# Ignaciagothe/tda-eeg-audio

Measured on AMD Instinct MI355X. Metric: windows/sec end-to-end (dist->Rips H0/H1->Wasserstein), 47-ch EEG, higher is better.
Workload: dtype f64; 1 GPU; configs[4]+configs[2]: 1416 recordings x 5 bands x 15 selected windows = 106200 (EEG 47x250 f64, audio 250 f64) window pairs per pass, the whole job; per pair corr->dist->Rips H0/H1 (EEG 47 pts), tau per recording-band, Takens dim 3 sub 2 + Rips (audio, 23..123 pts over the bands), Wasserstein H0+H1, features, per-recording reductions; one all-gather of the (1416, 5x48) rows per pass; windows_per_pass=106200, windows_per_gpu_per_pass=106200, input_bytes_per_gpu=10195200000, batches_per_pass=1, windows_per_batch=106200, parallelism=recordings dealt over 1 rank(s), one all-gather per pass, batches_in_flight=3, hip_graph=True, batches_rerun_with_full_ladder=0

## Files before the change

### tda_eeg_audio_amd/csrc/rips.hip

```cpp
#include "common.h"
#include "corr_dist_dev.h"
#include <stdlib.h>

#ifndef CLOUD_NB
#define CLOUD_NB 8192
#endif
#ifndef NARROW_NT
#define NARROW_NT 512
#endif
#ifndef NARROW_WAVES
#define NARROW_WAVES 6
#endif
#if defined(TDA_PROFILE) && !defined(TDA_PROFILE_STOPS_ONLY)
#define NARROW_NB (NARROW_NT == 384 ? 1536 : 1024)
#else
#define NARROW_NB (NARROW_NT == 384 ? 1536 : 2048)
#endif
#define NARROW_EMAX 7626
#define NT_MAX 512
#define RANK_NONE 0x7fffu

#ifdef TDA_PROFILE
__device__ unsigned long long g_prof[48];
#ifdef TDA_PROFILE_STOPS_ONLY
// ... 82 lines not shown
{
    WT o = 0;
#pragma unroll
    for (int i = 0; i < W; ++i) o |= a.w[i];
    return o != 0;
}
template <int W, typename WT>
__device__ __forceinline__ Psi<W, WT> pzero()
{
    Psi<W, WT> r;
#pragma unroll
    for (int i = 0; i < W; ++i) r.w[i] = 0;
    return r;
}

__device__ __forceinline__ double wave_min_f64(double v)
{
#pragma unroll
    for (int off = 32; off > 0; off >>= 1) { const double o = __shfl_xor(v, off, 64); v = o < v ? o : v; }
    return v;
}
__device__ __forceinline__ double wave_max_f64(double v)
{
#pragma unroll
    for (int off = 32; off > 0; off >>= 1) { const double o = __shfl_xor(v, off, 64); v = o > v ? o : v; }
    return v;
}

__device__ __forceinline__ int tri2(int v) { return (v * (v - 1)) >> 1; }
__device__ __forceinline__ int pair_index(int x, int y) { return x > y ? tri2(x) + y : tri2(y) + x; }

__device__ __forceinline__ int edge_row(int e)
{
    const int a = (int)((1.0f + __builtin_amdgcn_sqrtf(1.0f + 8.0f * (float)e)) * 0.5f);
    const int t = tri2(a);
    return a + (t + a <= e ? 1 : 0) - (t > e ? 1 : 0);
}

#ifndef TDA_NO_EDGE_TABLE
struct EdgeTable {
    u16 v[8192 + 512];
    constexpr EdgeTable() : v()
    {
        int a = 1, b = 0;
        for (int e = 0; e < 8192 + 512; ++e) { v[e] = (u16)((a << 8) | b); if (++b == a) { ++a; b = 0; } }
    }
};
__device__ const EdgeTable g_edge_ab = EdgeTable();
__device__ __forceinline__ u32 edge_ab(int e) { return (u32)g_edge_ab.v[e]; }
#else
__device__ __forceinline__ u32 edge_ab(int e) { const int a = edge_row(e); return (u32)((a << 8) | (e - tri2(a))); }
#endif

struct WgVote {
    u32* slots;
    int parity;
};
template <int NT>
__device__ __forceinline__ bool wg_any(WgVote& v, bool p)
{
    static_assert(NT % 64 == 0 && NT <= 512, "slots are read as one or two 16-byte words; slots beyond NT / 64 hold zero");
    const bool w = __ballot(p) != 0ull;
    u32* s = v.slots + 8 * v.parity;
    if ((threadIdx.x & 63) == 0) s[threadIdx.x >> 6] = w ? 1u : 0u;
    __syncthreads();
    v.parity ^= 1;
    const uint4 x = *reinterpret_cast<const uint4*>(s);
    u32 r = x.x | x.y | x.z | x.w;
    if (NT > 256) { const uint4 y = *reinterpret_cast<const uint4*>(s + 4); r |= y.x | y.y | y.z | y.w; }
    return r != 0u;
}
template <int NT>
__device__ __forceinline__ bool wg_all(WgVote& v, bool p) { return !wg_any<NT>(v, !p); }

__device__ __forceinline__ int wave_incl_scan_i32(int v)
{
#define TDA_DPP_ADD_(CTRL, RM) v += __builtin_amdgcn_update_dpp(0, v, CTRL, RM, 0xF, true)
    TDA_DPP_ADD_(0x111, 0xF);
    TDA_DPP_ADD_(0x112, 0xF);
    TDA_DPP_ADD_(0x114, 0xF);
    TDA_DPP_ADD_(0x118, 0xF);
    TDA_DPP_ADD_(0x142, 0xA);
    TDA_DPP_ADD_(0x143, 0xC);
#undef TDA_DPP_ADD_
    return v;
}

__device__ __forceinline__ int edge_flat(u32 pk) { return tri2((int)(pk >> 8)) + (int)(pk & 255u); }

struct Bucketer {
    float dmin, scale, top;
    __device__ __forceinline__ int operator()(u32 key) const
    {
        const float x = fminf((sortable_f32(key) - dmin) * scale, top);
        const int b = (int)x;
        return b < 0 ? 0 : b;
    }
};

template <int NT>
__device__ __forceinline__ void effective_threshold(int n, u32 tkey, const u32* vmax, u32 kmin_thread, u32* red, u32& teff_out, u32& kmin_out)
{
    const int tid = threadIdx.x;
    const int lane = tid & 63;
    const u32 m0 = lane < n ? vmax[lane] : 0xffffffffu, m1 = lane + 64 < n ? vmax[lane + 64] : 0xffffffffu;
    const u32 renc = wave_min_u32_dpp(m0 < m1 ? m0 : m1);
    teff_out = renc < tkey ? renc : tkey;
    if (tid == 0) red[1] = 0xffffffffu;
    __syncthreads();
    const u32 kmin = wave_min_u32_dpp(kmin_thread);
    if (lane == 63) atomicMin(&red[1], kmin);
    __syncthreads();
    kmin_out = red[1];
}

template <int NT, int NB, bool WANT_KEYS>
__device__ __forceinline__ int rank_edges(const u32* key32, int E, u32 teff, u32 kmin, u16* members, u32* cursor, int* wsum, u16* rank,
                          u16* ord, u32* skey)
{
    static_assert(NB % (2 * NT) == 0, "every thread scans whole words");
    constexpr int WPT = NB / NT / 2;
    const int tid = threadIdx.x, lane = tid & 63, wave = tid >> 6;
    Bucketer bk;
    bk.dmin = sortable_f32(kmin);
    bk.top = (float)(NB - 1);
    bk.scale = bk.top / (sortable_f32(teff) - bk.dmin);
    for (int i = tid; i < NB / 2; i += NT) cursor[i] = 0u;
    __syncthreads();
#pragma unroll 4
    for (int e = tid; e < E; e += NT) {
        const u32 k = key32[e];
        u32 b = 0xffffu;
        if (k <= teff) { b = (u32)bk(k); atomicAdd(&cursor[b >> 1], 1u << (16 * (b & 1))); }
        rank[e] = (u16)b;
    }
    __syncthreads();
    {
        u32 w[WPT];
        int s = 0;
#pragma unroll
        for (int i = 0; i < WPT; ++i) {
// ... 205 lines not shown
#endif
#define TDA_SOLO_BEGIN() __builtin_amdgcn_s_setprio(TDA_SOLO_PRIO)
#define TDA_SOLO_END() __builtin_amdgcn_s_setprio(0)

#define TDA_POLL_LIMIT (1 << 16)
#ifndef TDA_TURN_SLEEP
#define TDA_TURN_SLEEP 4
#endif
#ifdef TDA_DEBUG_PTS
__device__ int g_fault;
extern "C" __attribute__((visibility("default"))) int tda_debug_inject(int what)
{
    return hipMemcpyToSymbol(HIP_SYMBOL(g_fault), &what, sizeof(int)) != hipSuccess;
}
#define TDA_FAULT(n) (g_fault == (n))
#else
#define TDA_FAULT(n) false
#endif
#ifdef TDA_DEBUG_PTS
#define GUARD_BYTES 16
__device__ __forceinline__ void guard_write(unsigned char* smem, const RipsLayout& L)
{
    if ((int)threadIdx.x < 4 * L.n_guard) reinterpret_cast<u32*>(smem + L.guard[threadIdx.x >> 2] - GUARD_BYTES)[threadIdx.x & 3] = 0xC0FFEE00u + threadIdx.x;
    __syncthreads();
}
__device__ __forceinline__ int guard_check(unsigned char* smem, const RipsLayout& L)
{
    __syncthreads();
    bool bad = false;
    if ((int)threadIdx.x < 4 * L.n_guard) bad = reinterpret_cast<u32*>(smem + L.guard[threadIdx.x >> 2] - GUARD_BYTES)[threadIdx.x & 3] != 0xC0FFEE00u + threadIdx.x;
    return __syncthreads_or(bad ? 1 : 0) ? TDA_WIN_LDS_GUARD : 0;
}
#else
#define GUARD_BYTES 0
__device__ __forceinline__ void guard_write(unsigned char*, const RipsLayout&) {}
__device__ __forceinline__ int guard_check(unsigned char*, const RipsLayout&) { return 0; }
#endif

#define MISC_COMP 0
#define MISC_CAND 512
#define MISC_WV (512 + 128)
#define MISC_MIN (512 + 192)
#define MISC_DONE (512 + 208)
#define MISC_SORTCNT (512 + 224)
#define MISC_SHARED (MISC_DONE + NT_MAX)
#define MISC_CKEY (MISC_SHARED + 96)
#define MISC_LIST MISC_CKEY
#define MISC_LIST_BYTES (4 * NT_MAX + 1280)
#define MISC_ADJ (MISC_LIST + MISC_LIST_BYTES)
#define MISC_ADJC (MISC_ADJ + 128 * 16)
#define MISC_BRANK (MISC_ADJC + 128 * 16)
#define MISC_BYTES(ncls) (MISC_BRANK + 8 * (ncls))

template <int NT, int NVW, int W, typename WT, bool NARROW, class KEYFN>
__device__ __forceinline__ void rips_sweep(int n, int E, int Ev, const u16* rank, const u16* ord, Psi<W, WT>* psi, int psi_bytes,
                           unsigned char* misc, KEYFN keyfn, double* h0, int h0_cap, double* h1, int h1_cap,
                           int& out_k0, int& out_k1, int& out_status)
{
    static_assert(!NARROW || W == 1, "the narrow layout is the point-cloud first pass");
    int psi_cap = 0;
    const int tid0 = threadIdx.x;
    const int lane0 = tid0 & 63, wave = uni(tid0 >> 6);
    int* brank = reinterpret_cast<int*>(misc + MISC_BRANK);
    u64* cand = reinterpret_cast<u64*>(misc + MISC_CAND);
    unsigned char* done = misc + MISC_DONE;
    SweepShared* shared = reinterpret_cast<SweepShared*>(misc + MISC_SHARED);
    u64* adj = reinterpret_cast<u64*>(misc + MISC_ADJ);
    constexpr int WB = 8 * (int)sizeof(WT);
    float* bkey = reinterpret_cast<float*>(misc + MISC_BRANK + 4 * WB * W);
    u64* adjc = reinterpret_cast<u64*>(misc + MISC_ADJC);

    if constexpr (!NARROW) for (int e = tid0; e < E; e += NT) psi[e] = pzero<W, WT>();
    for (int i = tid0; i < WB * W; i += NT) { brank[i] = -1; bkey[i] = 0.f; }
    for (int i = tid0; i < 256; i += NT) { adj[i] = 0ull; adjc[i] = 0ull; }
    if (tid0 == 0) {
        u32* lc = reinterpret_cast<u32*>(misc + MISC_MIN);
        lc[0] = 0u; lc[1] = 0xffffffffu; lc[2] = 0u;
        lc[3] = 0u;
        shared->status = 0;
    }
    if (tid0 < 16) {
        reinterpret_cast<u32*>(misc + MISC_WV)[tid0] = 0u;
        cand[tid0] = 0ull;
    }
    __syncthreads();

    WgVote vote{reinterpret_cast<u32*>(misc + MISC_WV), 0};
    WT alive[W];
#pragma unroll
    for (int c = 0; c < W; ++c) alive[c] = 0;
    int k0 = 0, k1 = 0, merges = 0, status = 0;
    int compA = lane0, compB = lane0 + 64;

    int clen = NT;
    int ordcls = 0;
    int cov_next = tid0;
#ifdef TDA_PROFILE
    int prof_rneed = 0, prof_chunk = -1;
#endif
    PROF_RESUME();
    for (int r0 = 0; r0 < Ev && !status; r0 += clen) {
        int tid = tid0;
        LAUNDER(tid);
        const int lane = tid & 63;
        clen = NT;
        PROF_MARK(15);
#ifdef TDA_PROFILE
        ++prof_chunk;
#endif
        PROF_COUNT(23, 1);
        const int r = r0 + tid;
        const bool valid = r < Ev;
        int a = 1, b = 0;
        if (valid) { const u32 pk = ord[r]; a = (int)(pk >> 8); b = (int)(pk & 255u); }
        const int tab = tri2(a) + b;
        const int slot = NARROW ? r : tab;
        if constexpr (NARROW) {
            psi_cap = (psi_bytes - 2 * (E - r0)) >> 2;
            if (r < psi_cap) psi[r] = pzero<W, WT>();
        }
        u64 M[NVW], M0[NVW];
        u64 Aj[NVW], Bj[NVW];
#pragma unroll
        for (int w = 0; w < NVW; ++w) { M[w] = 0; M0[w] = 0; Aj[w] = 0; Bj[w] = 0; }
        if (valid) {
#pragma unroll
            for (int w = 0; w < NVW; ++w) { Aj[w] = adj[2 * a + w]; Bj[w] = adj[2 * b + w]; M0[w] = Aj[w] & Bj[w]; }
        }
        {
            volatile u32* turn = reinterpret_cast<volatile u32*>(misc + MISC_MIN) + 2;
            if (wave > 0) {
                int trips = 0;
                for (;;) {
                    const u32 t = (u32)uni((int)*turn);
                    if (t >= (u32)wave) break;
                    if (++trips > TDA_POLL_LIMIT) { if (lane == 0) turn[1] = 1u; break; }
                    if (t + 1u < (u32)wave) __builtin_amdgcn_s_sleep(TDA_TURN_SLEEP); else __builtin_amdgcn_s_sleep(0);
                }
            }
            __builtin_amdgcn_fence(__ATOMIC_ACQUIRE, "workgroup");
            if (valid) {
#pragma unroll
                for (int w = 0; w < NVW; ++w) M[w] = (Aj[w] | adjc[2 * a + w]) & (Bj[w] | adjc[2 * b + w]);
                atomicOr(reinterpret_cast<unsigned long long*>(&adjc[2 * a + (b >> 6)]), 1ull << (b & 63));
                atomicOr(reinterpret_cast<unsigned long long*>(&adjc[2 * b + (a >> 6)]), 1ull << (a & 63));
            }
            LDS_ORDER();
            if (lane == 0 && !(TDA_FAULT(1) && wave == 3)) *turn = (u32)wave + 1u;
        }
        if (valid) {
            const int ta0 = tri2(a), tb0 = tri2(b);
#pragma unroll
            for (int w = 0; w < NVW; ++w) {
                u64 cc = (Aj[w] | adjc[2 * a + w]) & (Bj[w] | adjc[2 * b + w]) & ~M[w];
                while (cc) {
                    const int v0 = 64 * w + __builtin_ctzll(cc); cc &= cc - 1ull;
                    const bool ok1 = cc != 0ull; const int v1 = ok1 ? 64 * w + __builtin_ctzll(cc) : v0; cc &= cc - 1ull;
                    const int t0 = tri2(v0), t1 = tri2(v1);
                    const u32 xa0 = rank[v0 < a ? ta0 + v0 : t0 + a], xb0 = rank[v0 < b ? tb0 + v0 : t0 + b];
                    const u32 xa1 = rank[v1 < a ? ta0 + v1 : t1 + a], xb1 = rank[v1 < b ? tb0 + v1 : t1 + b];
                    if ((int)(xa0 > xb0 ? xa0 : xb0) < r) M[w] |= 1ull << (v0 & 63);
                    if (ok1 && (int)(xa1 > xb1 ? xa1 : xb1) < r) M[w] |= 1ull << (v1 & 63);
                }
            }
        }
        u64 many = 0;
#pragma unroll
        for (int w = 0; w < NVW; ++w) many |= M[w];
        const bool is_cand = valid && many == 0;
        int vstar = 0, d1 = 0, d2 = 0, q1 = 0, q2 = 0;
        {
            u64 many0 = 0;
#pragma unroll
            for (int w = 0; w < NVW; ++w) many0 |= M0[w];
            if (many0) {
                if (NVW == 1 || M0[0]) vstar = __builtin_ctzll(M0[0]);
                else vstar = 64 + __builtin_ctzll(M0[NVW - 1]);
            } else if (many) {
                if (NVW == 1 || M[0]) vstar = __builtin_ctzll(M[0]);
                else vstar = 64 + __builtin_ctzll(M[NVW - 1]);
            }
            if (valid && many != 0) {
                d1 = pair_index(a, vstar); d2 = pair_index(b, vstar);
                q1 = (int)rank[d1] - r0; q2 = (int)rank[d2] - r0;
                if (TDA_FAULT(2) && tid == 77 && q1 >= 0) q1 = tid;
            }
        }
        PROF_MARK(4);
        PROF_STOPC(11, out_k0 = k0; out_k1 = k1; out_status = 0);
        u64* mbal = reinterpret_cast<u64*>(misc + MISC_COMP);
        u64* zbal = mbal + 8;
        int* offs = reinterpret_cast<int*>(mbal + 16);
        u16* freebits = reinterpret_cast<u16*>(misc + MISC_CKEY);
        float mykey = 0.f;
        if (is_cand) mykey = keyfn(r, a, b);
        {
            const u64 bal = __ballot(is_cand), zb = __ballot(is_cand && mykey == 0.0f);
            if (lane == 0) { cand[wave] = bal; zbal[wave] = zb; }
        }
        done[tid] = 0;
        __syncthreads();
        PROF_MARK(21);
        PROF_STOPC(12, out_k0 = k0; out_k1 = k1; out_status = 0);
        int nfree = 0;
#pragma unroll
        for (int c = 0; c < W; ++c) nfree += __builtin_popcountll((u64)(WT)~alive[c]);
        int ncand = 0;
#pragma unroll
        for (int w = 0; w < NT / 64; ++w) ncand += __builtin_popcountll(cand[w]);
        int btot = 0;
        if (ncand > 0) {
        const bool par = ncand > 24;
        const int lblA0 = compA, lblB0 = compB;
        int qpar = NT;
        if (par) {
            int* bcomp = reinterpret_cast<int*>(misc + MISC_LIST + 1024);
            u32* bbest2 = reinterpret_cast<u32*>(bcomp + 128);
            int* bpar = reinterpret_cast<int*>(bcomp + 384);
            auto rounds = [&](int limit) {
                if (wave == 0) { bcomp[lane] = lblA0; bcomp[64 + lane] = lblB0; }
                if (tid < 256) bbest2[tid] = 0xffffffffu;
                __syncthreads();
                bool live = is_cand && tid < limit, picked = false;
                for (int round = 0; round < 64; ++round) {
                    u32* bbest = bbest2 + 128 * (round & 1);
                    int ca = 0, cb2 = 0;
                    if (live) {
                        ca = bcomp[a]; cb2 = bcomp[b];
                        if (ca == cb2) live = false;
                        else { atomicMin(&bbest[ca], (u32)tid); atomicMin(&bbest[cb2], (u32)tid); }
                    }
                    if (!wg_any<NT>(vote, live)) break;
                    if (live && (bbest[ca] == (u32)tid || bbest[cb2] == (u32)tid)) { picked = true; live = false; }
                    if (wave == 0) {
                        TDA_SOLO_BEGIN();
                        int pp[2];
#pragma unroll
                        for (int h = 0; h < 2; ++h) {
                            const int me = lane + 64 * h;
                            pp[h] = me;
                            const u32 bp = bbest[me];
                            if (bp != 0xffffffffu) {
                                const u32 pk = ord[r0 + (int)bp];
                                const int oa = bcomp[pk >> 8], ob = bcomp[pk & 255u];
                                pp[h] = oa == me ? ob : oa;
                                if (bbest[pp[h]] == bp && me < pp[h]) pp[h] = me;
                            }
                        }
                        bpar[lane] = pp[0]; bpar[64 + lane] = pp[1];
                        for (int it = 0; it < 8; ++it) {
                            const int p0 = bpar[lane], p1 = bpar[64 + lane];
                            const int g0 = bpar[p0], g1 = bpar[p1];
                            if (__ballot(g0 != p0 || g1 != p1) == 0ull) break;
                            bpar[lane] = g0; bpar[64 + lane] = g1;
                        }
                        const int c0 = bcomp[lane], c1 = bcomp[64 + lane];
                        const int n0 = bpar[c0], n1 = bpar[c1];
                        bcomp[lane] = n0; bcomp[64 + lane] = n1;
                        u32* other = bbest2 + 128 * ((round + 1) & 1);
                        other[lane] = 0xffffffffu; other[64 + lane] = 0xffffffffu;
                        TDA_SOLO_END();
                    }
                    __syncthreads();
                }
                const u64 mb = __ballot(picked);
                if (lane == 0) mbal[wave] = mb;
                __syncthreads();
            };
            rounds(NT);
            int nbirth = 0, wcut = -1, before = 0;
#pragma unroll
            for (int w = 0; w < NT / 64; ++w) {
                const int nb = __builtin_popcountll(cand[w] & ~mbal[w]);
                if (wcut < 0 && nbirth + nb > nfree) { wcut = w; before = nbirth; }
                nbirth += nb;
            }
            if (wcut >= 0) {
                u64 bw = cand[wcut] & ~mbal[wcut];
                for (int k = before; k < nfree; ++k) bw &= bw - 1ull;
                qpar = 64 * wcut + __builtin_ctzll(bw);
                PROF_COUNT(26, 1);
                __syncthreads();
                rounds(qpar);
            }
            if (wave == 0) { compA = bcomp[lane]; compB = bcomp[64 + lane]; }
        }
        if (wave == 0) {
            TDA_SOLO_BEGIN();
            const u64 candv = cand[lane & 7];
            int q = par ? qpar : NT, births = 0;
            const bool walk = !par;
            for (int g = 0; g < NT / 64 && walk; ++g) {
                u64 cb = q == NT ? rl64(candv, g) : 0ull;
                u64 mm = 0ull;
                if (cb) {
                    PROF_COUNT(20, __builtin_popcountll(cb));
                    const u32 pkv = ord[r0 + 64 * g + lane < E ? r0 + 64 * g + lane : E - 1];
                    while (cb) {
                        const int l = __builtin_ctzll(cb);
                        cb &= cb - 1;
                        const u32 pk = rl32(pkv, l);
                        const int qa = (int)(pk >> 8), qb = (int)(pk & 255u);
                        int ca, cbb;
                        if (NVW == 1) {
                            ca = (int)rl32((u32)compA, qa);
                            cbb = (int)rl32((u32)compA, qb);
                        } else {
                            const int a0 = (int)rl32((u32)compA, qa & 63), a1 = (int)rl32((u32)compB, qa & 63);
                            const int b0 = (int)rl32((u32)compA, qb & 63), b1 = (int)rl32((u32)compB, qb & 63);
                            ca = qa < 64 ? a0 : a1;
                            cbb = qb < 64 ? b0 : b1;
                        }
                        const bool same = ca == cbb, open = q == NT;
                        q = (open && same && births == nfree) ? 64 * g + l : q;
                        births += same ? 1 : 0;
                        const int cnew = (q == NT) ? ca : cbb;
                        compA = compA == cbb ? cnew : compA;
                        if (NVW == 2) compB = compB == cbb ? cnew : compB;
                        mm |= (!same && q == NT) ? (1ull << l) : 0ull;
                    }
                }
                if (lane == 0) mbal[g] = mm;
            }
            int nb = 0, nr = 0, nm = 0;
            if (lane < NT / 64) {
                u64 cg = cand[lane];
                if (64 * lane >= q) cg = 0ull;
                else if (q < 64 * lane + 64) cg &= (1ull << (q - 64 * lane)) - 1ull;
                const u64 mg = mbal[lane], zg = zbal[lane];
                nb = __builtin_popcountll(cg & ~mg); nr = __builtin_popcountll(mg & ~zg); nm = __builtin_popcountll(mg);
            }
            int pb = 0, pr = 0, tb = 0, tr = 0, tm = 0;
#pragma unroll
            for (int w = 0; w < NT / 64; ++w) {
                const int xb = (int)rl32((u32)nb, w), xr = (int)rl32((u32)nr, w), xm = (int)rl32((u32)nm, w);
                if (w < lane) { pb += xb; pr += xr; }
                tb += xb; tr += xr; tm += xm;
            }
            if (lane < NT / 64) { offs[lane] = pb; offs[8 + lane] = pr; }
            if (lane == 0) { offs[16] = tb; offs[17] = tr; offs[18] = tm; offs[19] = q; }
            TDA_SOLO_END();
        } else {
            for (int t = tid - 64; t < WB * W; t += NT - 64) {
                const int cw = t / WB, bit = t & (WB - 1);
                int rk = 0;
                bool fr = false;
#pragma unroll
                for (int c = 0; c < W; ++c) {
                    const WT f_ = (WT)~alive[c];
                    if (c < cw) rk += __builtin_popcountll((u64)f_);
                    if (c == cw) { rk += __builtin_popcountll((u64)(f_ & (((WT)1 << bit) - (WT)1))); fr = (f_ >> bit) & (WT)1; }
                }
                if (fr) freebits[rk] = (u16)t;
            }
        }
        __syncthreads();
        PROF_MARK(22);
        PROF_STOPC(13, out_k0 = k0; out_k1 = k1; out_status = 0);
        clen = uni(offs[19]);
        if (clen == 0) status |= TDA_WIN_CLASS_OVERFLOW;
        if (clen < NT) PROF_COUNT(14, 1);
        bool mrg = is_cand && ((mbal[wave] >> lane) & 1ull);
        bool birth = is_cand && !mrg && tid < clen;
        bool row = mrg && mykey != 0.0f;
        const u64 below = (1ull << lane) - 1ull;
        const int bpre = offs[wave] + __builtin_popcountll(__ballot(birth) & below);
        const int rpre = offs[8 + wave] + __builtin_popcountll(__ballot(row) & below);
        btot = uni(offs[16]);
        const int rtot = uni(offs[17]), mtot = uni(offs[18]);
        if (!status) {
            if (row) {
                const int pos = k0 + rpre;
                if (pos < h0_cap) { h0[2 * pos] = 0.0; h0[2 * pos + 1] = (double)mykey; }
            }
            k0 += rtot; merges += mtot;
            if (birth) {
                const int idx = (int)freebits[bpre];
                const int cw = idx / WB, bit = idx & (WB - 1);
                Psi<W, WT> nv = pzero<W, WT>();
#pragma unroll
                for (int c = 0; c < W; ++c)
                    if (c == cw) nv.w[c] = ((WT)1 << bit);
                if (!NARROW || r < psi_cap) psi[slot] = nv;
                brank[idx] = r;
                bkey[idx] = mykey;
            }
            if (W == 1 && wave == 0 && btot > 0) {
                const int nal = __builtin_popcountll((u64)alive[0]);
                if (lane >= nal && lane < nal + btot) ordcls = (int)freebits[lane - nal];
            }
            int left = btot;
#pragma unroll
            for (int c = 0; c < W; ++c) {
                const u64 f_ = (u64)(WT)~alive[c];
                const int pc = __builtin_popcountll(f_);
                if (left >= pc) { alive[c] = (WT)~(WT)0; left -= pc; }
                else if (left > 0) {
                    int lo = 0, hi = 63;
                    while (lo < hi) {
                        const int mid = (lo + hi) >> 1;
                        if (__builtin_popcountll(f_ & ((2ull << mid) - 1ull)) >= left) hi = mid; else lo = mid + 1;
                    }
                    alive[c] |= (WT)(f_ & ((2ull << lo) - 1ull));
                    left = 0;
                }
            }
        }
        }
        if (status) break;
        PROF_MARK(5);
        PROF_STOPC(14, out_k0 = k0; out_k1 = k1; out_status = 0);
        bool quiet = btot == 0;
#pragma unroll
        for (int c = 0; c < W; ++c) quiet = quiet && alive[c] == 0;
        u32* lcnt = reinterpret_cast<u32*>(misc + MISC_MIN);
        if (quiet) PROF_COUNT(24, 1);
#ifdef TDA_PROFILE
        if (!quiet) prof_rneed = r0 + clen;
#endif
        if constexpr (NARROW) {
            if (!quiet && r0 + NT > psi_cap) { status |= TDA_WIN_CLASS_OVERFLOW; break; }
        }
// ... 318 lines not shown
                    if (nk == KMAX) { more = 1; break; }
                    const int src = __builtin_ctzll(__ballot(mk == best));
                    Psi<W, WT> mine = pzero<W, WT>();
#pragma unroll
                    for (int q = 0; q < LPL; ++q)
                        if (q < nq && ek[q] == best) mine = ev[q];
                    Psi<W, WT> wv;
#pragma unroll
                    for (int c = 0; c < W; ++c) {
                        if (sizeof(WT) == 8) wv.w[c] = (WT)rl64((u64)mine.w[c], src);
                        else wv.w[c] = (WT)rl32((u32)mine.w[c], src);
                    }
                    const int rk = r0 + (int)(best >> 8);
                    int ybit, ycw;
                    float ybirth;
                    if (W == 1) {
                        const u64 ob = __ballot(lane < nalive0 && (((u64)wv.w[0] >> ordcls) & 1ull));
                        if (!ob) { status |= TDA_WIN_CLASS_OVERFLOW; break; }
                        const int opos = 63 - __builtin_clzll(ob);
                        ybit = (int)rl32((u32)ordcls, opos);
                        ycw = 0;
                        ybirth = __uint_as_float(rl32(__float_as_uint(bky[0]), ybit));
                        const int up = __builtin_amdgcn_update_dpp(0, ordcls, 0x130, 0xF, 0xF, true);
                        if (lane >= opos) ordcls = up;
                        --nalive0;
                    } else {
                        int candv = -1, cwl = 0;
                        float byl = 0.f;
#pragma unroll
                        for (int c = 0; c < W; ++c)
                            if (lane < WB && ((wv.w[c] >> lb) & (WT)1) && brk[c] > candv) { candv = brk[c]; cwl = c; byl = bky[c]; }
                        const int bestr = wave_max_i32_dpp(candv);
                        const u64 ybal = __ballot(candv == bestr && candv >= 0);
                        if (!ybal) { status |= TDA_WIN_CLASS_OVERFLOW; break; }
                        ybit = __builtin_ctzll(ybal);
                        ycw = (int)rl32((u32)cwl, ybit);
                        ybirth = __uint_as_float(rl32(__float_as_uint(byl), ybit));
                    }
                    if (FTAB) {
                        WT sel = 0;
#pragma unroll
                        for (int c = 0; c < W; ++c)
                            if (c == ycw) sel = (vimg.w[c] >> ybit) & (WT)1;
                        if (lane < nk && sel) vimg = pxor(vimg, wv);
                        if (lane == nk) {
                            vimg = wv;
#pragma unroll
                            for (int c = 0; c < W; ++c)
                                if (c == ycw) vimg.w[c] &= (WT)~((WT)1 << ybit);
                            mycode = ((u32)ycw << 8) | (u32)ybit; myrk = (u32)rk; mybirth = ybirth;
                        }
                    } else {
                        const u32 pkk = ord[rk];
                        const float key = keyfn(rk, (int)(pkk >> 8), (int)(pkk & 255u));
                        if (key > ybirth) {
                            if (k1 < h1_cap && lane == 0) { h1[2 * k1] = (double)ybirth; h1[2 * k1 + 1] = (double)key; }
                            ++k1;
                        }
                        if (lane == 0) {
                            *reinterpret_cast<u32*>(list + ES * nk) = ((u32)ycw << 8) | (u32)ybit;
#pragma unroll
                            for (int c = 0; c < W; ++c) *reinterpret_cast<WT*>(list + ES * nk + 4 + c * (int)sizeof(WT)) = wv.w[c];
                        }
                    }
#pragma unroll
                    for (int q = 0; q < LPL; ++q) {
                        if (q >= nq) break;
                        WT sel = 0;
#pragma unroll
                        for (int c = 0; c < W; ++c)
                            if (c == ycw) sel = (ev[q].w[c] >> ybit) & (WT)1;
                        if (sel) ev[q] = pxor(ev[q], wv);
                    }
#pragma unroll
                    for (int c = 0; c < W; ++c)
                        if (c == ycw) alive[c] &= (WT)~((WT)1 << ybit);
                    ++nk;
                }
                PROF_MARK(31);
                PROF_COUNT(10, nk);
                if (FTAB) {
                    const bool mine_ok = lane < nk;
                    float key = 0.f;
                    if (mine_ok) {
                        const u32 pkk = ord[(int)myrk];
                        key = keyfn((int)myrk, (int)(pkk >> 8), (int)(pkk & 255u));
                    }
                    const bool emit = mine_ok && key > mybirth;
                    const u64 bal = __ballot(emit);
                    const int pos = k1 + __builtin_popcountll(bal & ((1ull << lane) - 1ull));
                    if (emit && pos < h1_cap) { h1[2 * pos] = (double)mybirth; h1[2 * pos + 1] = (double)key; }
                    k1 += __builtin_popcountll(bal);
                    if (mine_ok) {
                        Psi<W, WT>* ftab = reinterpret_cast<Psi<W, WT>*>(list);
                        ftab[WB * (int)(mycode >> 8) + (int)(mycode & 255u)] = vimg;
                    }
                }
                if (lane == 0) {
#pragma unroll
                    for (int c = 0; c < W; ++c) shared->alive[c] = (u64)alive[c];
                    shared->k1 = k1; shared->nk = nk; shared->more = more; shared->status = status;
                }
                TDA_SOLO_END();
            }
            __syncthreads();
            PROF_MARK(18);
            PROF_STOPC(18, out_k0 = k0; out_k1 = k1; out_status = 0);
            WT kmask[W];
#pragma unroll
            for (int c = 0; c < W; ++c) {
                const WT na = sizeof(WT) == 8 ? (WT)uni64(shared->alive[c]) : (WT)uni((int)(u32)shared->alive[c]);
                kmask[c] = alive_before[c] & (WT)~na; alive[c] = na;
            }
            k1 = uni(shared->k1);
            const int nk = uni(shared->nk);
            const bool more = uni(shared->more) != 0;
            status = uni(shared->status);
            if (status) break;
            if (FTAB) {
                const Psi<W, WT>* ftab = reinterpret_cast<const Psi<W, WT>*>(list);
                const int seen_end = r0 + clen < Ev ? r0 + clen : Ev;
#pragma unroll 4
                for (int rr = tid; rr < seen_end; rr += NT) {
                    const int e = NARROW ? rr : edge_flat(ord[rr]);
                    const Psi<W, WT> p = psi[e];
                    WT anyh = 0;
#pragma unroll
                    for (int c = 0; c < W; ++c) anyh |= p.w[c] & kmask[c];
                    if (!anyh) continue;
                    Psi<W, WT> q;
#pragma unroll
                    for (int c = 0; c < W; ++c) q.w[c] = p.w[c] & (WT)~kmask[c];
#pragma unroll
                    for (int c = 0; c < W; ++c) {
                        u64 hh = (u64)(p.w[c] & kmask[c]);
                        while (hh) {
                            const int bit = __builtin_ctzll(hh);
                            hh &= hh - 1ull;
                            q = pxor(q, ftab[WB * c + bit]);
// ... 6 lines not shown
                    u32 kc[4];
                    Psi<W, WT> kw[4];
#pragma unroll
                    for (int j = 0; j < 4; ++j) {
                        const int jj = j0 + j < nk ? j0 + j : j0;
                        kc[j] = j0 + j < nk ? *reinterpret_cast<const u32*>(list + ES * jj) : 0xffffffffu;
#pragma unroll
                        for (int c = 0; c < W; ++c) kw[j].w[c] = *reinterpret_cast<const WT*>(list + ES * jj + 4 + c * (int)sizeof(WT));
                    }
#pragma unroll 4
                    for (int rr = tid; rr < (r0 + clen < Ev ? r0 + clen : Ev); rr += NT) {
                        const int e = NARROW ? rr : edge_flat(ord[rr]);
                        Psi<W, WT> p = psi[e];
                        bool changed = false;
#pragma unroll
                        for (int j = 0; j < 4; ++j) {
                            if (kc[j] == 0xffffffffu) continue;
                            const int jcw = (int)(kc[j] >> 8), jbit = (int)(kc[j] & 255u);
                            WT sel = 0;
#pragma unroll
                            for (int c = 0; c < W; ++c)
                                if (c == jcw) sel = (p.w[c] >> jbit) & (WT)1;
                            if (sel) { p = pxor(p, kw[j]); changed = true; }
                        }
                        if (changed) psi[e] = p;
                    }
                }
            }
            PROF_MARK(19);
            PROF_STOPC(19, out_k0 = k0; out_k1 = k1; out_status = 0);
            if (complete && !more) break;
            if (++list_rounds > 4 * NT) { status |= TDA_WIN_CLASS_OVERFLOW; break; }
            __syncthreads();
        }
        }
        if (valid && tid < clen) {
            atomicOr(reinterpret_cast<unsigned long long*>(&adj[2 * a + (b >> 6)]), 1ull << (b & 63));
            atomicOr(reinterpret_cast<unsigned long long*>(&adj[2 * b + (a >> 6)]), 1ull << (a & 63));
        }
        if (tid < 256) adjc[tid] = 0ull;
        if (tid == 0) {
            lcnt[0] = 0u; lcnt[1] = 0xffffffffu; lcnt[2] = 0u; shared->clen = 0x7fffffff;
            if (lcnt[3]) shared->status = TDA_WIN_NOT_CONVERGED;
        }
        __syncthreads();
        if (uni(shared->status) & TDA_WIN_NOT_CONVERGED) { status |= TDA_WIN_NOT_CONVERGED; break; }
        if (quiet) {
            const int from = r0 + clen;
            bool covered = true;
            int rr = (NT & (NT - 1)) == 0 ? from + ((tid - from) & (NT - 1)) : from + (((tid - from) % NT) + NT) % NT;
            rr = rr > cov_next ? rr : cov_next;
            while (rr < Ev) {
                const u32 pk = ord[rr];
                const int ea = (int)(pk >> 8), eb = (int)(pk & 255u);
                u64 common = adj[2 * ea] & adj[2 * eb];
                if (NVW == 2) common |= adj[2 * ea + 1] & adj[2 * eb + 1];
                if (common == 0ull) { covered = false; break; }
                rr += NT;
            }
            cov_next = rr;
            {
                const u32 wmin = wave_min_u32_dpp(covered ? 0x7fffffffu : (u32)rr);
                if (lane == 0 && wmin != 0x7fffffffu) atomicMin(reinterpret_cast<unsigned int*>(&shared->clen), wmin);
            }
            __syncthreads();
            const int ru = uni(shared->clen);
            if (ru >= Ev) { PROF_COUNT(25, 1); PROF_MARK(7); break; }
            if (ru > from) {
                for (int r2 = from + tid; r2 < ru; r2 += NT) {
                    const u32 pk = ord[r2];
                    const int ea = (int)(pk >> 8), eb = (int)(pk & 255u);
                    atomicOr(reinterpret_cast<unsigned long long*>(&adj[2 * ea + (eb >> 6)]), 1ull << (eb & 63));
                    atomicOr(reinterpret_cast<unsigned long long*>(&adj[2 * eb + (ea >> 6)]), 1ull << (ea & 63));
                    if constexpr (NARROW) { if (r2 < ((psi_bytes - 2 * (E - ru)) >> 2)) psi[r2] = pzero<W, WT>(); }
                }
                PROF_COUNT(35, ru - from);
                clen = ru - r0;
                __syncthreads();
            }
        }
        PROF_MARK(7);
        PROF_STOPC(20, out_k0 = k0; out_k1 = k1; out_status = 0);
    }
#ifdef TDA_PROFILE
    PROF_COUNT(36, prof_rneed > 4096 ? 1 : 0); PROF_COUNT(37, prof_rneed > 4608 ? 1 : 0); PROF_COUNT(38, prof_rneed > 5120 ? 1 : 0);
    PROF_COUNT(39, prof_rneed); PROF_COUNT(40, Ev);
#endif
    const int ncomp = n - merges;
    for (int i = 0; i < ncomp; ++i) {
        if (k0 < h0_cap && tid0 == 0) { h0[2 * k0] = 0.0; h0[2 * k0 + 1] = (double)INFINITY; }
        ++k0;
    }
#pragma unroll
    for (int c = 0; c < W; ++c) {
        u64 al = (u64)alive[c];
        while (al) {
            const int bit = __builtin_ctzll(al);
            al &= al - 1;
            if (k1 < h1_cap && tid0 == 0) { h1[2 * k1] = (double)bkey[WB * c + bit]; h1[2 * k1 + 1] = (double)INFINITY; }
            ++k1;
        }
    }
    if (k1 > h1_cap) status |= TDA_WIN_H1_TRUNCATED;
    out_k0 = k0; out_k1 = k1; out_status = status;
}


#define TOT_NW 128
#define TOT_SLOTS 8
#define TOT_SLOT_WORDS ((size_t)8128 * TOT_NW)

template <int NT, class KEYFN>
__device__ __forceinline__ void rips_sweep_total(int n, int E, int Ev, const u16* rank, const u16* ord, float* bkey, unsigned char* misc,
                                 u64* __restrict__ psi_g, KEYFN keyfn, double* h0, int h0_cap, double* h1, int h1_cap,
                                 int& out_k0, int& out_k1, int& out_status)
{
    constexpr int NWV = NT / 64;
    const int tid = threadIdx.x, lane = tid & 63, wave = uni(tid >> 6);
    u64* adj = reinterpret_cast<u64*>(misc + MISC_ADJ);
    int* comp = reinterpret_cast<int*>(misc + MISC_COMP);
    u32* flags = reinterpret_cast<u32*>(misc + MISC_WV);
    u64* yv = reinterpret_cast<u64*>(misc + MISC_LIST);
    u64* cur = yv + TOT_NW;
    u32* nzbit = reinterpret_cast<u32*>(misc + MISC_ADJ + 4096);
    u32* alivebit = nzbit + 256;
    static_assert(MISC_LIST_BYTES >= 2 * TOT_NW * 8, "scratch of the total sweep");
    for (int i = tid; i < 256; i += NT) { adj[i] = 0ull; nzbit[i] = 0u; alivebit[i] = 0u; }
    for (int v = tid; v < 128; v += NT) comp[v] = v;
    __syncthreads();
    int k0 = 0, k1 = 0, merges = 0, nborn = 0, nalive = 0;
    auto stored = [&](int rr) { return (nzbit[rr >> 5] >> (rr & 31)) & 1u; };
    for (int r = 0; r < Ev; ++r) {
        const u32 pk = (u32)uni((int)ord[r]);
        const int a = (int)(pk >> 8), b = (int)(pk & 255u);
        const u64 M0 = uni64(adj[2 * a] & adj[2 * b]), M1 = uni64(adj[2 * a + 1] & adj[2 * b + 1]);
        if ((M0 | M1) == 0ull) {
            const int ca = uni(comp[a]), cb = uni(comp[b]);
            const float key = keyfn(r, a, b);
            __syncthreads();
// ... 975 lines not shown
```

Baseline: 4.153 million windows/s.

## Precompute H0 spanning forest via Boruvka before sweep, drop per-chunk merge detection

```diff
diff --git a/tda_eeg_audio_amd/csrc/rips.hip b/tda_eeg_audio_amd/csrc/rips.hip
--- a/tda_eeg_audio_amd/csrc/rips.hip
+++ b/tda_eeg_audio_amd/csrc/rips.hip
@@ -158,27 +158,6 @@
 __device__ __forceinline__ u32 edge_ab(int e) { const int a = edge_row(e); return (u32)((a << 8) | (e - tri2(a))); }
 #endif
 
-struct WgVote {
-    u32* slots;
-    int parity;
-};
-template <int NT>
-__device__ __forceinline__ bool wg_any(WgVote& v, bool p)
-{
-    static_assert(NT % 64 == 0 && NT <= 512, "slots are read as one or two 16-byte words; slots beyond NT / 64 hold zero");
-    const bool w = __ballot(p) != 0ull;
-    u32* s = v.slots + 8 * v.parity;
-    if ((threadIdx.x & 63) == 0) s[threadIdx.x >> 6] = w ? 1u : 0u;
-    __syncthreads();
-    v.parity ^= 1;
-    const uint4 x = *reinterpret_cast<const uint4*>(s);
-    u32 r = x.x | x.y | x.z | x.w;
-    if (NT > 256) { const uint4 y = *reinterpret_cast<const uint4*>(s + 4); r |= y.x | y.y | y.z | y.w; }
-    return r != 0u;
-}
-template <int NT>
-__device__ __forceinline__ bool wg_all(WgVote& v, bool p) { return !wg_any<NT>(v, !p); }
-
 __device__ __forceinline__ int wave_incl_scan_i32(int v)
 {
 #define TDA_DPP_ADD_(CTRL, RM) v += __builtin_amdgcn_update_dpp(0, v, CTRL, RM, 0xF, true)
@@ -192,7 +171,7 @@
     return v;
 }
 
-__device__ __forceinline__ int edge_flat(u32 pk) { return tri2((int)(pk >> 8)) + (int)(pk & 255u); }
+__device__ __forceinline__ int edge_flat(u32 pk) { return tri2((int)((pk >> 8) & 127u)) + (int)(pk & 255u); }
 
 struct Bucketer {
     float dmin, scale, top;
@@ -504,17 +483,141 @@
 #define MISC_BRANK (MISC_ADJC + 128 * 16)
 #define MISC_BYTES(ncls) (MISC_BRANK + 8 * (ncls))
 
+#define TDA_WIN_FOREST_GUARD 0x200
+#define ORD_FOREST 0x8000u
+
+typedef unsigned short u16x2 __attribute__((ext_vector_type(2)));
+typedef short i16x2 __attribute__((ext_vector_type(2)));
+__device__ __forceinline__ u16x2 as_u16x2(u32 x) { return __builtin_bit_cast(u16x2, x); }
+
+template <int NT, int NVW>
+__device__ __forceinline__ int spanning_forest(int n, const u16* rank, u16* ord, unsigned char* misc)
+{
+    constexpr int NV = 64 * NVW;
+    constexpr int TPV = (NT / NV) >= 8 ? 8 : (NT / NV) >= 4 ? 4 : (NT / NV) >= 2 ? 2 : 1;
+    constexpr int UPT = NV / TPV;
+    static_assert(NT >= NV && UPT % 4 == 0, "one thread per vertex at least, whole label words");
+    unsigned char* flab = misc + MISC_LIST + 1024;
+    u32* fbest = reinterpret_cast<u32*>(flab + 128);
+    int* fhook = reinterpret_cast<int*>(flab + 640);
+    const int tid = threadIdx.x, lane = tid & 63, wave = tid >> 6;
+    const int v = tid / TPV, j = tid & (TPV - 1);
+    if (tid < 128) { flab[tid] = (unsigned char)tid; fbest[tid] = 0xffffffffu; }
+    u32 row[UPT / 2];
+    {
+        const int tv = tri2(v), u0 = UPT * j;
+        int tu = tri2(u0);
+#pragma unroll
+        for (int i = 0; i < UPT; ++i) {
+            const int u = u0 + i;
+            const bool ok = v < n && u < n && u != v;
+            const u32 rk = rank[ok ? (u < v ? tv + u : tu + v) : 0];
+            const u32 x = ok ? rk : RANK_NONE;
+            if (i & 1) row[i >> 1] |= x << 16; else row[i >> 1] = x;
+            tu += u;
+        }
+    }
+    __syncthreads();
+    int ncomp = n;
+    for (int round = 0; ncomp > 1; ++round) {
+        if (v < n) {
+            const int cv = flab[v];
+            u16x2 acc = {0xffffu, 0xffffu};
+            if (round == 0) {
+#pragma unroll
+                for (int k = 0; k < UPT / 2; ++k) acc = __builtin_elementwise_min(acc, as_u16x2(row[k]));
+            } else {
+                const u32 cv4 = (u32)cv * 0x01010101u;
+#pragma unroll
+                for (int k = 0; k < UPT / 4; ++k) {
+                    const u32 x4 = reinterpret_cast<const u32*>(flab + UPT * j)[k] ^ cv4;
+#pragma unroll
+                    for (int h = 0; h < 2; ++h) {
+                        const u16x2 d = as_u16x2(__builtin_amdgcn_perm(0u, x4, h ? 0x0c030c02u : 0x0c010c00u));
+                        const u16x2 one = {1u, 1u};
+                        const i16x2 same = __builtin_bit_cast(i16x2, (u16x2)(d - one)) >> (short)15;
+                        acc = __builtin_elementwise_min(acc, as_u16x2(row[2 * k + h] | __builtin_bit_cast(u32, same)));
+                    }
+                }
+            }
+            u32 m = acc.x < acc.y ? acc.x : acc.y;
+#pragma unroll
+            for (int s = 1; s < TPV; s <<= 1) {
+                const u32 o = (u32)__shfl_xor((int)m, s);
+                m = o < m ? o : m;
+            }
+            if (j == 0 && m < RANK_NONE) atomicMin(&fbest[cv], m);
+        }
+        __syncthreads();
+        if (wave == 0) {
+            TDA_SOLO_BEGIN();
+            int c[NVW], p[NVW];
+            bool hook[NVW];
+#pragma unroll
+            for (int h = 0; h < NVW; ++h) {
+                const int me = lane + 64 * h;
+                c[h] = flab[me];
+                p[h] = me;
+                hook[h] = false;
+                const u32 bm = fbest[me];
+                if (c[h] == me && bm != 0xffffffffu) {
+                    const u32 pk = ord[bm];
+                    const int la = flab[(pk >> 8) & 127u], lb = flab[pk & 255u];
+                    const int o = la == me ? lb : la;
+                    const bool root = fbest[o] == bm && me < o;
+                    if (!root) {
+                        p[h] = o;
+                        ord[bm] = (u16)(pk | ORD_FOREST);
+                        hook[h] = true;
+                    }
+                }
+            }
+#pragma unroll
+            for (int h = 0; h < NVW; ++h) fbest[lane + 64 * h] = 0xffffffffu;
+            for (;;) {
+                int g[NVW];
+                bool moved = false;
+#pragma unroll
+                for (int h = 0; h < NVW; ++h) {
+                    g[h] = __shfl(p[0], p[h] & 63);
+                    if (NVW == 2) { const int g1 = __shfl(p[NVW - 1], p[h] & 63); g[h] = p[h] < 64 ? g[h] : g1; }
+                    moved = moved || g[h] != p[h];
+                }
+                if (__ballot(moved) == 0ull) break;
+#pragma unroll
+                for (int h = 0; h < NVW; ++h) p[h] = g[h];
+            }
+#pragma unroll
+            for (int h = 0; h < NVW; ++h) {
+                int nc = __shfl(p[0], c[h] & 63);
+                if (NVW == 2) { const int n1 = __shfl(p[NVW - 1], c[h] & 63); nc = c[h] < 64 ? nc : n1; }
+                flab[lane + 64 * h] = (unsigned char)nc;
+            }
+            int hooks = 0;
+#pragma unroll
+            for (int h = 0; h < NVW; ++h) hooks += __builtin_popcountll(__ballot(hook[h]));
+            if (lane == 0) *fhook = hooks;
+            TDA_SOLO_END();
+        }
+        __syncthreads();
+        const int hooks = uni(*fhook);
+        PROF_COUNT(42, 1);
+        if (hooks == 0) break;
+        ncomp -= hooks;
+    }
+    return ncomp;
+}
+
 template <int NT, int NVW, int W, typename WT, bool NARROW, class KEYFN>
-__device__ __forceinline__ void rips_sweep(int n, int E, int Ev, const u16* rank, const u16* ord, Psi<W, WT>* psi, int psi_bytes,
+__device__ __forceinline__ void rips_sweep(int n, int E, int Ev, const u16* rank, u16* ord, Psi<W, WT>* psi, int psi_bytes,
                            unsigned char* misc, KEYFN keyfn, double* h0, int h0_cap, double* h1, int h1_cap,
                            int& out_k0, int& out_k1, int& out_status)
 {
     static_assert(!NARROW || W == 1, "the narrow layout is the point-cloud first pass");
     int psi_cap = 0;
     const int tid0 = threadIdx.x;
-    const int lane0 = tid0 & 63, wave = uni(tid0 >> 6);
+    const int wave = uni(tid0 >> 6);
     int* brank = reinterpret_cast<int*>(misc + MISC_BRANK);
-    u64* cand = reinterpret_cast<u64*>(misc + MISC_CAND);
     unsigned char* done = misc + MISC_DONE;
     SweepShared* shared = reinterpret_cast<SweepShared*>(misc + MISC_SHARED);
     u64* adj = reinterpret_cast<u64*>(misc + MISC_ADJ);
@@ -531,18 +634,12 @@
         lc[3] = 0u;
         shared->status = 0;
     }
-    if (tid0 < 16) {
-        reinterpret_cast<u32*>(misc + MISC_WV)[tid0] = 0u;
-        cand[tid0] = 0ull;
-    }
-    __syncthreads();
-
-    WgVote vote{reinterpret_cast<u32*>(misc + MISC_WV), 0};
+    __syncthreads();
+
     WT alive[W];
 #pragma unroll
     for (int c = 0; c < W; ++c) alive[c] = 0;
     int k0 = 0, k1 = 0, merges = 0, status = 0;
-    int compA = lane0, compB = lane0 + 64;
 
     int clen = NT;
     int ordcls = 0;
@@ -551,6 +648,12 @@
     int prof_rneed = 0, prof_chunk = -1;
 #endif
     PROF_RESUME();
+    const int fcomps = spanning_forest<NT, NVW>(n, rank, ord, misc);
+    (void)fcomps;
+#ifdef TDA_DEBUG_PTS
+    bool fguard = false;
+#endif
+    PROF_MARK(41);
     for (int r0 = 0; r0 < Ev && !status; r0 += clen) {
         int tid = tid0;
         LAUNDER(tid);
@@ -564,7 +667,8 @@
         const int r = r0 + tid;
         const bool valid = r < Ev;
         int a = 1, b = 0;
-        if (valid) { const u32 pk = ord[r]; a = (int)(pk >> 8); b = (int)(pk & 255u); }
+        bool forest = false;
+        if (valid) { const u32 pk = ord[r]; a = (int)((pk >> 8) & 127u); b = (int)(pk & 255u); forest = (pk & ORD_FOREST) != 0u; }
         const int tab = tri2(a) + b;
         const int slot = NARROW ? r : tab;
         if constexpr (NARROW) {
@@ -640,15 +744,31 @@
         }
         PROF_MARK(4);
         PROF_STOPC(11, out_k0 = k0; out_k1 = k1; out_status = 0);
-        u64* mbal = reinterpret_cast<u64*>(misc + MISC_COMP);
-        u64* zbal = mbal + 8;
-        int* offs = reinterpret_cast<int*>(mbal + 16);
+        u64* bbal = reinterpret_cast<u64*>(misc + MISC_COMP);
+        u64* rbal = bbal + 8;
+        u64* mbal = bbal + 16;
         u16* freebits = reinterpret_cast<u16*>(misc + MISC_CKEY);
         float mykey = 0.f;
         if (is_cand) mykey = keyfn(r, a, b);
+        const bool fmrg = valid && forest, fbirth = is_cand && !forest;
+#ifdef TDA_DEBUG_PTS
+        fguard = fguard || (fmrg && !is_cand);
+#endif
         {
-            const u64 bal = __ballot(is_cand), zb = __ballot(is_cand && mykey == 0.0f);
-            if (lane == 0) { cand[wave] = bal; zbal[wave] = zb; }
+            const u64 bb = __ballot(fbirth), rb = __ballot(fmrg && mykey != 0.0f), mb = __ballot(fmrg);
+            if (lane == 0) { bbal[wave] = bb; rbal[wave] = rb; mbal[wave] = mb; }
+        }
+        for (int t = tid; t < WB * W; t += NT) {
+            const int cw = t / WB, bit = t & (WB - 1);
+            int rk = 0;
+            bool fr = false;
+#pragma unroll
+            for (int c = 0; c < W; ++c) {
+                const WT f_ = (WT)~alive[c];
+                if (c < cw) rk += __builtin_popcountll((u64)f_);
+                if (c == cw) { rk += __builtin_popcountll((u64)(f_ & (((WT)1 << bit) - (WT)1))); fr = (f_ >> bit) & (WT)1; }
+            }
+            if (fr) freebits[rk] = (u16)t;
         }
         done[tid] = 0;
         __syncthreads();
@@ -657,169 +777,38 @@
         int nfree = 0;
 #pragma unroll
         for (int c = 0; c < W; ++c) nfree += __builtin_popcountll((u64)(WT)~alive[c]);
-        int ncand = 0;
-#pragma unroll
-        for (int w = 0; w < NT / 64; ++w) ncand += __builtin_popcountll(cand[w]);
+        const int wl = lane < NT / 64 ? lane : 0;
+        const u64 bv = lane < NT / 64 ? bbal[wl] : 0ull, rv = lane < NT / 64 ? rbal[wl] : 0ull, mv = lane < NT / 64 ? mbal[wl] : 0ull;
+        const int nbl = __builtin_popcountll(bv);
+        const int ibl = wave_incl_scan_i32(nbl);
+        const int nball = (int)rl32((u32)ibl, NT / 64 - 1);
         int btot = 0;
-        if (ncand > 0) {
-        const bool par = ncand > 24;
-        const int lblA0 = compA, lblB0 = compB;
-        int qpar = NT;
-        if (par) {
-            int* bcomp = reinterpret_cast<int*>(misc + MISC_LIST + 1024);
-            u32* bbest2 = reinterpret_cast<u32*>(bcomp + 128);
-            int* bpar = reinterpret_cast<int*>(bcomp + 384);
-            auto rounds = [&](int limit) {
-                if (wave == 0) { bcomp[lane] = lblA0; bcomp[64 + lane] = lblB0; }
-                if (tid < 256) bbest2[tid] = 0xffffffffu;
-                __syncthreads();
-                bool live = is_cand && tid < limit, picked = false;
-                for (int round = 0; round < 64; ++round) {
-                    u32* bbest = bbest2 + 128 * (round & 1);
-                    int ca = 0, cb2 = 0;
-                    if (live) {
-                        ca = bcomp[a]; cb2 = bcomp[b];
-                        if (ca == cb2) live = false;
-                        else { atomicMin(&bbest[ca], (u32)tid); atomicMin(&bbest[cb2], (u32)tid); }
-                    }
-                    if (!wg_any<NT>(vote, live)) break;
-                    if (live && (bbest[ca] == (u32)tid || bbest[cb2] == (u32)tid)) { picked = true; live = false; }
-                    if (wave == 0) {
-                        TDA_SOLO_BEGIN();
-                        int pp[2];
-#pragma unroll
-                        for (int h = 0; h < 2; ++h) {
-                            const int me = lane + 64 * h;
-                            pp[h] = me;
-                            const u32 bp = bbest[me];
-                            if (bp != 0xffffffffu) {
-                                const u32 pk = ord[r0 + (int)bp];
-                                const int oa = bcomp[pk >> 8], ob = bcomp[pk & 255u];
-                                pp[h] = oa == me ? ob : oa;
-                                if (bbest[pp[h]] == bp && me < pp[h]) pp[h] = me;
-                            }
-                        }
-                        bpar[lane] = pp[0]; bpar[64 + lane] = pp[1];
-                        for (int it = 0; it < 8; ++it) {
-                            const int p0 = bpar[lane], p1 = bpar[64 + lane];
-                            const int g0 = bpar[p0], g1 = bpar[p1];
-                            if (__ballot(g0 != p0 || g1 != p1) == 0ull) break;
-                            bpar[lane] = g0; bpar[64 + lane] = g1;
-                        }
-                        const int c0 = bcomp[lane], c1 = bcomp[64 + lane];
-                        const int n0 = bpar[c0], n1 = bpar[c1];
-                        bcomp[lane] = n0; bcomp[64 + lane] = n1;
-                        u32* other = bbest2 + 128 * ((round + 1) & 1);
-                        other[lane] = 0xffffffffu; other[64 + lane] = 0xffffffffu;
-                        TDA_SOLO_END();
-                    }
-                    __syncthreads();
-                }
-                const u64 mb = __ballot(picked);
-                if (lane == 0) mbal[wave] = mb;
-                __syncthreads();
-            };
-            rounds(NT);
-            int nbirth = 0, wcut = -1, before = 0;
-#pragma unroll
-            for (int w = 0; w < NT / 64; ++w) {
-                const int nb = __builtin_popcountll(cand[w] & ~mbal[w]);
-                if (wcut < 0 && nbirth + nb > nfree) { wcut = w; before = nbirth; }
-                nbirth += nb;
-            }
-            if (wcut >= 0) {
-                u64 bw = cand[wcut] & ~mbal[wcut];
-                for (int k = before; k < nfree; ++k) bw &= bw - 1ull;
-                qpar = 64 * wcut + __builtin_ctzll(bw);
-                PROF_COUNT(26, 1);
-                __syncthreads();
-                rounds(qpar);
-            }
-            if (wave == 0) { compA = bcomp[lane]; compB = bcomp[64 + lane]; }
-        }
-        if (wave == 0) {
-            TDA_SOLO_BEGIN();
-            const u64 candv = cand[lane & 7];
-            int q = par ? qpar : NT, births = 0;
-            const bool walk = !par;
-            for (int g = 0; g < NT / 64 && walk; ++g) {
-                u64 cb = q == NT ? rl64(candv, g) : 0ull;
-                u64 mm = 0ull;
-                if (cb) {
-                    PROF_COUNT(20, __builtin_popcountll(cb));
-                    const u32 pkv = ord[r0 + 64 * g + lane < E ? r0 + 64 * g + lane : E - 1];
-                    while (cb) {
-                        const int l = __builtin_ctzll(cb);
-                        cb &= cb - 1;
-                        const u32 pk = rl32(pkv, l);
-                        const int qa = (int)(pk >> 8), qb = (int)(pk & 255u);
-                        int ca, cbb;
-                        if (NVW == 1) {
-                            ca = (int)rl32((u32)compA, qa);
-                            cbb = (int)rl32((u32)compA, qb);
-                        } else {
-                            const int a0 = (int)rl32((u32)compA, qa & 63), a1 = (int)rl32((u32)compB, qa & 63);
-                            const int b0 = (int)rl32((u32)compA, qb & 63), b1 = (int)rl32((u32)compB, qb & 63);
-                            ca = qa < 64 ? a0 : a1;
-                            cbb = qb < 64 ? b0 : b1;
-                        }
-                        const bool same = ca == cbb, open = q == NT;
-                        q = (open && same && births == nfree) ? 64 * g + l : q;
-                        births += same ? 1 : 0;
-                        const int cnew = (q == NT) ? ca : cbb;
-                        compA = compA == cbb ? cnew : compA;
-                        if (NVW == 2) compB = compB == cbb ? cnew : compB;
-                        mm |= (!same && q == NT) ? (1ull << l) : 0ull;
-                    }
-                }
-                if (lane == 0) mbal[g] = mm;
-            }
-            int nb = 0, nr = 0, nm = 0;
-            if (lane < NT / 64) {
-                u64 cg = cand[lane];
-                if (64 * lane >= q) cg = 0ull;
-                else if (q < 64 * lane + 64) cg &= (1ull << (q - 64 * lane)) - 1ull;
-                const u64 mg = mbal[lane], zg = zbal[lane];
-                nb = __builtin_popcountll(cg & ~mg); nr = __builtin_popcountll(mg & ~zg); nm = __builtin_popcountll(mg);
-            }
-            int pb = 0, pr = 0, tb = 0, tr = 0, tm = 0;
-#pragma unroll
-            for (int w = 0; w < NT / 64; ++w) {
-                const int xb = (int)rl32((u32)nb, w), xr = (int)rl32((u32)nr, w), xm = (int)rl32((u32)nm, w);
-                if (w < lane) { pb += xb; pr += xr; }
-                tb += xb; tr += xr; tm += xm;
-            }
-            if (lane < NT / 64) { offs[lane] = pb; offs[8 + lane] = pr; }
-            if (lane == 0) { offs[16] = tb; offs[17] = tr; offs[18] = tm; offs[19] = q; }
-            TDA_SOLO_END();
-        } else {
-            for (int t = tid - 64; t < WB * W; t += NT - 64) {
-                const int cw = t / WB, bit = t & (WB - 1);
-                int rk = 0;
-                bool fr = false;
-#pragma unroll
-                for (int c = 0; c < W; ++c) {
-                    const WT f_ = (WT)~alive[c];
-                    if (c < cw) rk += __builtin_popcountll((u64)f_);
-                    if (c == cw) { rk += __builtin_popcountll((u64)(f_ & (((WT)1 << bit) - (WT)1))); fr = (f_ >> bit) & (WT)1; }
-                }
-                if (fr) freebits[rk] = (u16)t;
-            }
-        }
-        __syncthreads();
+        if (nball > 0 || __ballot(mv != 0ull) != 0ull) {
+        int q = NT;
+        const u64 over = __ballot(lane < NT / 64 && ibl > nfree);
+        if (over) {
+            const int wcut = __builtin_ctzll(over);
+            u64 bw = rl64(bv, wcut);
+            for (int k = (int)rl32((u32)(ibl - nbl), wcut); k < nfree; ++k) bw &= bw - 1ull;
+            q = 64 * wcut + __builtin_ctzll(bw);
+            PROF_COUNT(26, 1);
+        }
+        const u64 keep = 64 * lane + 64 <= q ? ~0ull : 64 * lane >= q ? 0ull : (1ull << (q - 64 * lane)) - 1ull;
+        const int pk3 = nbl | (__builtin_popcountll(rv & keep) << 10) | (__builtin_popcountll(mv & keep) << 20);
+        const int i3 = wave_incl_scan_i32(pk3);
+        const int before3 = wave > 0 ? (int)rl32((u32)i3, wave - 1) : 0, tot3 = (int)rl32((u32)i3, NT / 64 - 1);
+        const int pb = before3 & 1023, pr = (before3 >> 10) & 1023, rtot = (tot3 >> 10) & 1023, mtot = tot3 >> 20;
+        btot = over ? nfree : nball;
+        clen = q;
         PROF_MARK(22);
         PROF_STOPC(13, out_k0 = k0; out_k1 = k1; out_status = 0);
-        clen = uni(offs[19]);
         if (clen == 0) status |= TDA_WIN_CLASS_OVERFLOW;
         if (clen < NT) PROF_COUNT(14, 1);
-        bool mrg = is_cand && ((mbal[wave] >> lane) & 1ull);
-        bool birth = is_cand && !mrg && tid < clen;
-        bool row = mrg && mykey != 0.0f;
+        const bool birth = fbirth && tid < clen;
+        const bool row = fmrg && mykey != 0.0f && tid < clen;
         const u64 below = (1ull << lane) - 1ull;
-        const int bpre = offs[wave] + __builtin_popcountll(__ballot(birth) & below);
-        const int rpre = offs[8 + wave] + __builtin_popcountll(__ballot(row) & below);
-        btot = uni(offs[16]);
-        const int rtot = uni(offs[17]), mtot = uni(offs[18]);
+        const int bpre = pb + __builtin_popcountll(__ballot(birth) & below);
+        const int rpre = pr + __builtin_popcountll(__ballot(row) & below);
         if (!status) {
             if (row) {
                 const int pos = k0 + rpre;
@@ -1244,7 +1233,7 @@
                         }
                     } else {
                         const u32 pkk = ord[rk];
-                        const float key = keyfn(rk, (int)(pkk >> 8), (int)(pkk & 255u));
+                        const float key = keyfn(rk, (int)((pkk >> 8) & 127u), (int)(pkk & 255u));
                         if (key > ybirth) {
                             if (k1 < h1_cap && lane == 0) { h1[2 * k1] = (double)ybirth; h1[2 * k1 + 1] = (double)key; }
                             ++k1;
@@ -1276,7 +1265,7 @@
                     float key = 0.f;
                     if (mine_ok) {
                         const u32 pkk = ord[(int)myrk];
-                        key = keyfn((int)myrk, (int)(pkk >> 8), (int)(pkk & 255u));
+                        key = keyfn((int)myrk, (int)((pkk >> 8) & 127u), (int)(pkk & 255u));
                     }
                     const bool emit = mine_ok && key > mybirth;
                     const u64 bal = __ballot(emit);
@@ -1389,7 +1378,7 @@
             rr = rr > cov_next ? rr : cov_next;
             while (rr < Ev) {
                 const u32 pk = ord[rr];
-                const int ea = (int)(pk >> 8), eb = (int)(pk & 255u);
+                const int ea = (int)((pk >> 8) & 127u), eb = (int)(pk & 255u);
                 u64 common = adj[2 * ea] & adj[2 * eb];
                 if (NVW == 2) common |= adj[2 * ea + 1] & adj[2 * eb + 1];
                 if (common == 0ull) { covered = false; break; }
@@ -1406,7 +1395,7 @@
             if (ru > from) {
                 for (int r2 = from + tid; r2 < ru; r2 += NT) {
                     const u32 pk = ord[r2];
-                    const int ea = (int)(pk >> 8), eb = (int)(pk & 255u);
+                    const int ea = (int)((pk >> 8) & 127u), eb = (int)(pk & 255u);
                     atomicOr(reinterpret_cast<unsigned long long*>(&adj[2 * ea + (eb >> 6)]), 1ull << (eb & 63));
                     atomicOr(reinterpret_cast<unsigned long long*>(&adj[2 * eb + (ea >> 6)]), 1ull << (ea & 63));
                     if constexpr (NARROW) { if (r2 < ((psi_bytes - 2 * (E - ru)) >> 2)) psi[r2] = pzero<W, WT>(); }
@@ -1422,6 +1411,12 @@
 #ifdef TDA_PROFILE
     PROF_COUNT(36, prof_rneed > 4096 ? 1 : 0); PROF_COUNT(37, prof_rneed > 4608 ? 1 : 0); PROF_COUNT(38, prof_rneed > 5120 ? 1 : 0);
     PROF_COUNT(39, prof_rneed); PROF_COUNT(40, Ev);
+#endif
+#ifdef TDA_DEBUG_PTS
+    {
+        const bool bad = __syncthreads_or(fguard ? 1 : 0) != 0 || merges != n - fcomps;
+        if (!status && bad) status |= TDA_WIN_FOREST_GUARD;
+    }
 #endif
     const int ncomp = n - merges;
     for (int i = 0; i < ncomp; ++i) {
```

New measurement: 4.181 million windows/s, median of 6. About the same (+0.7%).
